# Entscheider/depthhead

Hardware: NVIDIA B200
Metric: frames/s, 640x480 depth, 10 trees depth 15, stride 5 (higher is better)
Workload: dtype f64

## Files before the change

depthhead_b200/api.py:

```python
from __future__ import annotations

import ctypes as C
from dataclasses import dataclass

import numpy as np

from . import capi


class IntrinsicMatrix:

    def __init__(self, mat):
        m = np.asarray(mat, np.float32)
        if m.size != 9:
            raise ValueError("IntrinsicMatrix needs 9 values")
        self.mat = np.ascontiguousarray(m.reshape(3, 3))

    @staticmethod
    def default_kinect_intrinsic() -> "IntrinsicMatrix":
        return IntrinsicMatrix([[560.0, 0.0, 320.0], [0.0, 560.0, 240.0], [0.0, 0.0, 1.0]])

    def _ptr(self):
        return capi.ptr(self.mat)

# ... 49 lines not shown
    def stage_ms(self) -> dict:
        a = np.zeros(capi.DH_N_STAGES, np.float32)
        capi.check(capi.load().dh_ctx_stage_ms(self._h, capi.ptr(a)))
        return dict(zip(capi.STAGES, a.tolist()))

    def counters(self) -> dict:
        a = np.zeros(capi.DH_N_COUNTERS, np.uint64)
        capi.check(capi.load().dh_ctx_counters(self._h, capi.ptr(a)))
        return dict(zip(capi.COUNTERS, (int(x) for x in a)))

    def tile_plan(self) -> dict:
        v = np.zeros(8, np.uint32)
        capi.check(capi.load().dh_debug_tile_plan(self._h, capi.ptr(v)))
        keys = ("patches_x", "patches_y", "tiles_x", "tiles_y", "tile_w", "tile_h", "smem_bytes", "threads")
        return {k: int(x) for k, x in zip(keys, v)}

    def debug_dims(self):
        a, b, c = C.c_uint32(), C.c_uint32(), C.c_uint32()
        capi.check(capi.load().dh_debug_dims(self._h, C.byref(a), C.byref(b), C.byref(c)))
        return a.value, b.value, c.value

    def debug_leaf_indices(self) -> np.ndarray:
        npx, npy, T = self.debug_dims()
        out = np.zeros((npx * npy, T), np.int32)
        capi.check(capi.load().dh_debug_leaf_indices(self._h, capi.ptr(out)))
        return out

    def debug_patches(self):
        npx, npy, _ = self.debug_dims()
        p3 = np.zeros((npx * npy, 3), np.float32)
# ... 250 lines not shown
```

depthhead_b200/capi.py:

```python
from __future__ import annotations

import ctypes as C
import os

import numpy as np

from . import _build

DH_OK, DH_E_JSON, DH_E_SHAPE, DH_E_CUDA, DH_E_ARG, DH_E_STATE = 0, -1, -2, -3, -4, -5
DH_DEPTH_HOST, DH_DEPTH_DEVICE = 0, 1
DH_N_STAGES, DH_N_COUNTERS = 7, 12
STAGES = ("h2d", "sat", "traverse", "gate", "vote", "meanshift", "d2h")
COUNTERS = ("frames", "patches", "valid_patches", "evals", "node_visits", "gate_patches", "hits",
            "centre_votes", "rot_votes", "launches", "meanshift_iters", "cube_rebuilds")


class DhError(RuntimeError):
    def __init__(self, code: int, msg: str):
        super().__init__("%s (code %d)" % (msg, code))
        self.code = code


class dh_result(C.Structure):
    _fields_ = [("mid_point", C.c_float * 3), ("_pad", C.c_uint32), ("rotation", C.c_double * 3),
# ... 78 lines not shown
    "dh_hough_image_raw": (C.c_int, [_vp, _vp, _vp, _u32, _u32, _vp, _vp]),
    "dh_build_hough_image": (C.c_int, [_vp, _vp, _vp, _u32, _u32, _vp, _vp]),
    "dh_predict_from2dhough": (C.c_int, [_vp, _vp, _vp, _u32, _u32, _vp, C.POINTER(dh_result)]),
    "dh_ctx_enable_stage_timing": (C.c_int, [_vp, C.c_int]),
    "dh_ctx_stage_ms": (C.c_int, [_vp, _vp]),
    "dh_ctx_counters": (C.c_int, [_vp, _vp]),
    "dh_ctx_enable_debug": (C.c_int, [_vp, C.c_int]),
    "dh_debug_dims": (C.c_int, [_vp, C.POINTER(_u32), C.POINTER(_u32), C.POINTER(_u32)]),
    "dh_debug_leaf_indices": (C.c_int, [_vp, _vp]),
    "dh_debug_patches": (C.c_int, [_vp, _vp, _vp]),
    "dh_debug_seeds": (C.c_int, [_vp, _vp, _vp, _vp, _vp]),
    "dh_debug_votes": (C.c_int, [_vp, C.c_int, _vp, _vp, C.POINTER(_u64), _vp, C.POINTER(_i32)]),
    "dh_debug_meanshift": (C.c_int, [_vp, C.c_int, _vp, C.POINTER(_u32)]),
    "dh_debug_meanshift_flags": (C.c_int, [_vp, _vp]),
    "dh_debug_tile_plan": (C.c_int, [_vp, _vp]),
    "dh_debug_leaf_static": (C.c_int, [_vp, _vp, _vp, _vp, _vp]),
}

_lib = None


def lib_path() -> str:
    return _build.LIB


def load():
    global _lib
    if _lib is not None:
        return _lib
    if os.environ.get("DH_NO_BUILD") != "1":
# ... 25 lines not shown
```

depthhead_b200/csrc/dh_capi.cu:

```cuda
#include <cstring>
#include <memory>
#include <new>
#include <algorithm>
#include <string>
#include <vector>

#include "../../include/depthhead_cuda.h"
#include "dh_ctx.hpp"
#include "dh_forest.hpp"
#include "dh_json.hpp"

struct dh_forest {
    std::unique_ptr<dh::HostForest> hf;
};
struct dh_ctx {
    std::unique_ptr<dh::Context> cx;
};

namespace {

thread_local std::string g_last_error = "";

int fail(int code, const std::string& msg) {
    g_last_error = msg;
// ... 273 lines not shown
int dh_train_split_level(dh_ctx* c, const dh_trainset* t, const uint32_t* sample_idx, const uint64_t* node_off, uint32_t n_nodes,
                         const int32_t* rects, const double* thr, uint8_t* bits) {
    return guarded([&] {
        REQUIRE(c && t && node_off && (n_nodes == 0 || (sample_idx && rects && thr && bits)), "dh_train_split_level: NULL argument");
        c->cx->train_split_level(*t->ts, sample_idx, node_off, n_nodes, rects, thr, bits);
    });
}
int dh_debug_tile_plan(dh_ctx* c, uint32_t plan[8]) {
    return guarded([&] {
        REQUIRE(c && plan, "dh_debug_tile_plan: NULL argument");
        const dh::TilePlan& t = c->cx->tile_plan();
        const uint32_t v[8] = {t.tpx, t.tpy, t.tiles_x, t.tiles_y, t.tw, t.th, t.smem_bytes, t.threads};
        std::memcpy(plan, v, sizeof(v));
    });
}
int dh_train_forest(dh_ctx* c, const dh_train_params* p, const uint16_t* patches, uint64_t n, const uint8_t* is_object,
                    const float* offsets, const double* rotations, dh_forest** out) {
    return guarded([&] {
        REQUIRE(c && p && patches && is_object && offsets && rotations && out, "dh_train_forest: NULL argument");
        *out = nullptr;
        std::unique_ptr<dh::HostForest> hf(c->cx->train_forest(*p, patches, n, is_object, offsets, rotations));
        *out = new dh_forest{std::move(hf)};
    });
}
int dh_train_learn(dh_ctx* c, const dh_train_params* p, uint32_t n_frames, uint32_t w, uint32_t h, const uint16_t* depth,
                   const uint8_t* mask, const float* K, const float* pos3d, const float* rot, dh_forest** out) {
    return guarded([&] {
        REQUIRE(c && p && out && (n_frames == 0 || (depth && mask && K && pos3d && rot)), "dh_train_learn: NULL argument");
        *out = nullptr;
        std::unique_ptr<dh::HostForest> hf(c->cx->train_learn(*p, n_frames, w, h, depth, mask, K, pos3d, rot));
// ... 131 lines not shown
```

depthhead_b200/csrc/dh_ctx.cu:

```cuda
#include "dh_ctx.hpp"

#include <algorithm>
#include <atomic>
#include <chrono>
#include <cmath>
#include <cstdio>
#include <cstdlib>
#include <cstring>
#include <thread>

namespace dh {

#define DH_CUDA(expr)                                                                                   \
    do {                                                                                                \
        cudaError_t _e = (expr);                                                                        \
        if (_e != cudaSuccess)                                                                          \
            throw ModelError(DH_E_CUDA, std::string(#expr) + ": " + cudaGetErrorString(_e));            \
    } while (0)

namespace {

template <typename T>
void dev_alloc(T*& p, size_t n) {
    p = nullptr;
// ... 61 lines not shown
    }
    DH_CUDA(cudaStreamCreateWithFlags(&copy_stream2_, cudaStreamNonBlocking));
    for (int i = 0; i < kStageSlots; ++i) {
        DH_CUDA(cudaEventCreateWithFlags(&ev_copied_[i], cudaEventDisableTiming));
        DH_CUDA(cudaEventCreateWithFlags(&ev_consumed_[i], cudaEventDisableTiming));
    }
    dev_alloc(d_counters_, DH_N_COUNTERS);
    DH_CUDA(cudaHostAlloc((void**)&h_fs_, sizeof(FrameState), cudaHostAllocDefault));
    DH_CUDA(cudaHostAlloc((void**)&h_counters_, sizeof(unsigned long long) * DH_N_COUNTERS, cudaHostAllocDefault));
    DH_CUDA(cudaHostAlloc((void**)&h_result1_, sizeof(dh_result), cudaHostAllocDefault));
    for (int i = 0; i < kEncSlots; ++i) DH_CUDA(cudaEventCreateWithFlags(&ev_enc_copied_[i], cudaEventDisableTiming));
    DH_CUDA(cudaEventCreateWithFlags(&ev_copy_tail_, cudaEventDisableTiming));
    if (const char* v = std::getenv("DH_HOST_ENCODE")) host_encode_ = *v ? (int)std::strtol(v, nullptr, 10) : -1;
    use_graphs_ = env_flag("DH_GRAPH", true);
    cube_clear_fused_ = env_flag("DH_CUBE_CLEAR_FUSED", true);
    gate_split_ = env_flag("DH_GATE_SPLIT", true);
    gate_split_min_ = env_u32("DH_GATE_SPLIT_MIN", 64);
    chunk_frames_ = env_u32("DH_CHUNK_FRAMES", 0);
    debug_sync_ = env_u32("DH_DEBUG_SYNC", 0) != 0;
    std::memset(stage_ms_, 0, sizeof(stage_ms_));
    std::memset(counters_, 0, sizeof(counters_));
}

Context::~Context() {
    cudaSetDevice(device_);
    cudaDeviceSynchronize();
    drop_graph();
    free_scratch();
    free_forest();
    dev_free(d_counters_);
// ... 272 lines not shown
    fdev_.pair_leaf_perm = df_pair_perm_;
    fdev_.leaf_prob = df_leaf_prob_;
    fdev_.leaf_info = df_leaf_info_;
    fdev_.offsets = df_offsets_;
    fdev_.rot_bins = df_rot_bins_;
    fdev_.rot_cells = df_rot_cells_;
    fdev_.leaf_box = df_leaf_box_;
    fdev_.ms_kernel = df_kernel_;
    fdev_.n_trees = hf.n_trees;
}

void Context::free_lane(Lane& L) {
    dev_free(L.sat);
    dev_free(L.band_u);
    dev_free(L.box);
    dev_free(L.leaf);
    dev_free(L.p3);
    dev_free(L.gate);
    dev_free(L.gated);
    dev_free(L.cubes);
    dev_free(L.grids);
    dev_free(L.fs);
    dev_free(L.results);
    dev_free(L.ms_trace);
    L.allocated = false;
    L.cubes_clean = false;
}

void Context::drop_graph() {
    if (graph_exec_) cudaGraphExecDestroy(graph_exec_);
// ... 21 lines not shown
        if (w + 1 <= 1024 && env_flag("DH_SAT_BANDS", true))
            dev_alloc(L.band_u, F * (size_t)((h + sat_band_rows() - 1) / sat_band_rows()) * (w + 1));
    }
    dev_alloc(L.leaf, F * P * T);
    dev_alloc(L.p3, F * P * 3);
    dev_alloc(L.gate, F * P);
    dev_alloc(L.gated, F * P);
    dev_alloc(L.cubes, F * 2 * (size_t)vote_box_cells());
    DH_CUDA(cudaMemsetAsync(L.cubes, 0, sizeof(uint32_t) * F * 2 * (size_t)vote_box_cells(), stream_));
    L.cubes_clean = true;
    dev_alloc(L.grids, F * (size_t)(kPosGridCells + kRotGridCells));
    dev_alloc(L.fs, F);
    dev_alloc(L.results, F);
    if (sk_.trace_iters) dev_alloc(L.ms_trace, F * 2 * (size_t)sk_.trace_iters * 3);
    if (g.P) {
        const cuuint64_t gdim[3] = {(cuuint64_t)(g.rw ? g.box_w : w + 1), (cuuint64_t)(g.rw ? g.box_h : h + 1), (cuuint64_t)F};
        const cuuint64_t row_bytes = (cuuint64_t)(g.rw ? g.box_pitch : g.sat_pitch) * 4u;
        const cuuint64_t gstr[2] = {row_bytes, row_bytes * (g.rw ? g.box_h : h + 1)};
        const cuuint32_t box[3] = {tiles_.tw, tiles_.th, 1u};
        const cuuint32_t estr[3] = {1u, 1u, 1u};
        CUresult r = get_encode_fn()(&L.sat_map, CU_TENSOR_MAP_DATA_TYPE_UINT32, 3, g.rw ? L.box : L.sat, gdim, gstr, box, estr,
                                     CU_TENSOR_MAP_INTERLEAVE_NONE, CU_TENSOR_MAP_SWIZZLE_NONE,
                                     CU_TENSOR_MAP_L2_PROMOTION_L2_128B, CU_TENSOR_MAP_FLOAT_OOB_FILL_NONE);
        if (r != CUDA_SUCCESS) throw ModelError(DH_E_CUDA, "cuTensorMapEncodeTiled failed with code " + std::to_string((int)r));
    }
    DH_CUDA(cudaStreamSynchronize(stream_));
    L.allocated = true;
}

TilePlan Context::plan_tiles(const Geometry& g) const {
// ... 124 lines not shown
        DH_CUDA(cudaStreamSynchronize(copy_stream_));
        DH_CUDA(cudaStreamSynchronize(copy_stream2_));
        for (int i = 0; i < kStageSlots; ++i) dev_free(d_depth_[i]);
        staging_elems_ = n;
    }
    for (int i = 0; i < slots && i < kStageSlots; ++i)
        if (!d_depth_[i]) dev_alloc(d_depth_[i], staging_elems_);
}

FrameBuffers Context::buffers(const Lane& L, const uint16_t* depth) const {
    FrameBuffers b{};
    b.depth = depth;
    b.sat = L.sat;
    b.band_u = L.band_u;
    b.box = L.box;
    b.leaf = L.leaf;
    b.p3 = debug_ ? L.p3 : nullptr;
    b.gate = debug_ ? L.gate : nullptr;
    b.gated = L.gated;
    b.grids = L.grids;
    b.fs = L.fs;
    b.cubes = L.cubes;
    b.results = L.results;
    b.ms_trace = L.ms_trace;
    b.ms_trace_cap = sk_.trace_iters;
    b.leaf_mask = leaf_codes_ ? kLeafIdMask : 0x7fffffffu;
    b.debug = debug_ ? 1u : 0u;
    b.clear_cubes = (!debug_ && cube_clear_fused_) ? 1u : 0u;
    return b;
}
// ... 36 lines not shown
    if (g.P && hot_tw_ != tiles_.tw) {
        launch_plan_nodes(df_nodes_, df_hot_, df_uni_, df_n_nodes_, tiles_.tw, leaf_codes_ ? df_leaf_prob_ : nullptr, stream_);
        if (df_pair_recs_) launch_plan_pairs(df_pair_topo_, df_uni_, df_pair_recs_, df_n_pairs_, stream_);
        DH_CUDA(cudaStreamSynchronize(stream_));
        hot_tw_ = tiles_.tw;
    }
    mark(DH_STAGE_SAT);
    launches_ += (uint64_t)(g.rw ? launch_box_image(b, g, n, n_sms_, st) : launch_sat(b, g, n, st));
    stage_check("sat");
    mark(DH_STAGE_TRAVERSE);
    if (g.P) {
        if (debug_)
            DH_CUDA(cudaMemsetAsync(L.leaf, 0xFF, sizeof(int32_t) * (size_t)n * g.n_trees * g.P, st));
        else
            DH_CUDA(cudaMemset2DAsync(L.leaf, sizeof(int32_t) * (size_t)g.n_trees * g.P, 0xFF, sizeof(int32_t) * (size_t)g.P, n, st));
        launch_traverse(L.sat_map, b, g, tiles_, fdev_, n, st);
        launches_ += 1;
        stage_check("traverse");
    }
}

void Context::run_back(Lane& L, const FrameBuffers& b, uint32_t n, uint32_t iterations) {
    const Geometry& g = geom_;
    cudaStream_t st = L.stream;
    mark(DH_STAGE_GATE);
    launches_ += (uint64_t)launch_gate_coarse(b, g, fdev_, n, gate_split_ && n >= gate_split_min_, n_sms_, st);
    stage_check("gate + coarse grids");
    mark(DH_STAGE_VOTE);
    if (iterations && !L.cubes_clean) DH_CUDA(cudaMemsetAsync(L.cubes, 0, sizeof(uint32_t) * 2 * (size_t)vote_box_cells() * n, st));
    if (iterations) L.cubes_clean = false;
    launches_ += (uint64_t)launch_seed_and_cubes(b, g, fdev_, n, iterations, st);
    stage_check("seeds + accumulator cubes");
// ... 706 lines not shown
    if (npx) *npx = geom_.npx;
    if (npy) *npy = geom_.npy;
    if (n_trees) *n_trees = geom_.n_trees;
}
void Context::debug_leaf(int32_t* leaf) {
    require_debug();
    const size_t P = geom_.P, T = geom_.n_trees;
    std::vector<int32_t> tmp(P * T);
    DH_CUDA(cudaMemcpy(tmp.data(), lanes_[0].leaf, P * T * sizeof(int32_t), cudaMemcpyDeviceToHost));
    for (size_t t = 0; t < T; ++t)
        for (size_t p = 0; p < P; ++p) {
            const int32_t w = tmp[t * P + p];
            leaf[p * T + t] = (w >= 0 && leaf_codes_) ? (int32_t)((uint32_t)w & kLeafIdMask) : w;
        }
}
void Context::debug_patches(float* p3, uint8_t* gate) {
    require_debug();
    const size_t P = geom_.P;
    if (gate) DH_CUDA(cudaMemcpy(gate, lanes_[0].gate, P, cudaMemcpyDeviceToHost));
    if (p3) DH_CUDA(cudaMemcpy(p3, lanes_[0].p3, P * 3 * sizeof(float), cudaMemcpyDeviceToHost));
}
void Context::debug_seeds(uint32_t* guess_pos, uint32_t* guess_rot, int32_t* seed_mid, int32_t* seed_rot) {
    require_debug();
    if (guess_pos) DH_CUDA(cudaMemcpy(guess_pos, lanes_[0].grids, kPosGridCells * sizeof(uint32_t), cudaMemcpyDeviceToHost));
    if (guess_rot) DH_CUDA(cudaMemcpy(guess_rot, lanes_[0].grids + kPosGridCells, kRotGridCells * sizeof(uint32_t), cudaMemcpyDeviceToHost));
    FrameState fs;
    DH_CUDA(cudaMemcpy(&fs, lanes_[0].fs, sizeof(fs), cudaMemcpyDeviceToHost));
    for (int k = 0; k < 3; ++k) {
        if (seed_mid) seed_mid[k] = fs.seed_mid[k];
        if (seed_rot) seed_rot[k] = fs.seed_rot[k];
// ... 61 lines not shown
```

depthhead_b200/csrc/dh_ctx.hpp:

```cpp
#pragma once

#include <cuda.h>
#include <cuda_runtime.h>

#include <cstdint>
#include <cstring>
#include <memory>
#include <utility>
#include <vector>

#include "dh_forest.hpp"
#include "dh_hostenc.hpp"
#include "dh_kernels.cuh"

namespace dh {

struct Lane {
    cudaStream_t stream = nullptr;
    cudaStream_t own = nullptr;
    cudaEvent_t done = nullptr;
    uint32_t* sat = nullptr;
    uint32_t* band_u = nullptr;
    uint32_t* box = nullptr;
    int32_t* leaf = nullptr;
    float* p3 = nullptr;
    uint8_t* gate = nullptr;
    float4* gated = nullptr;
    uint32_t* grids = nullptr;
    FrameState* fs = nullptr;
    dh_result* results = nullptr;
    int32_t* ms_trace = nullptr;
    uint32_t* cubes = nullptr;
    CUtensorMap sat_map{};
    bool allocated = false;
    bool cubes_clean = false;
};
constexpr int kMaxLanes = 4;

// ... 49 lines not shown
    void train_split_level(const TrainSet& ts, const uint32_t* sample_idx, const uint64_t* node_off, uint32_t n_nodes,
                           const int32_t* rects, const double* thr, uint8_t* bits);
    void predict_mask(const HostForest& hf, const uint16_t* depth, uint32_t w, uint32_t h, uint8_t* mask);
    void hough_image_raw(const HostForest& hf, const uint16_t* depth, uint32_t w, uint32_t h, const float K[9],
                         uint16_t* votes);
    void hough_image(const HostForest& hf, const uint16_t* depth, uint32_t w, uint32_t h, const float K[9], uint16_t* votes,
                     bool blur, dh_result* from2d);

    void debug_dims(uint32_t* npx, uint32_t* npy, uint32_t* n_trees) const;
    void debug_leaf(int32_t* leaf);
    void debug_patches(float* p3, uint8_t* gate);
    void debug_seeds(uint32_t* guess_pos, uint32_t* guess_rot, int32_t* seed_mid, int32_t* seed_rot);
    void debug_votes(int which, int32_t* keys, uint32_t* vals, uint64_t* n, int32_t* box_origin, int32_t* box_dim);
    void debug_meanshift(int which, int32_t* pos, uint32_t* n_iter);
    void debug_leaf_static(const HostForest& hf, uint32_t* valtoadd, uint8_t* rot_ok, uint8_t* off_ok);
    uint32_t last_ms_flags(int which) const { return last_ms_flags_[which & 1]; }
    const TilePlan& tile_plan() const { return tiles_; }

private:
    void ensure_forest(const HostForest& hf);
    void free_forest();
    void build_pair_tables(const HostForest& hf, const std::vector<int32_t>& dev_index);
    void ensure_scratch(const HostForest& hf, uint32_t w, uint32_t h, uint32_t n_frames_hint, const float K[9], int n_lanes = 1);
    void alloc_lane(Lane& L);
    void free_lane(Lane& L);
    void ensure_staging(int slots);
    void ensure_biwi(const uint64_t* offsets, uint32_t n, uint32_t chunk, int slots);
    void check_biwi_status(uint32_t n);
    void run_batch(const HostForest& hf, const uint16_t* depth, const uint8_t* blob, const uint64_t* offsets, uint32_t n, uint32_t w,
                   uint32_t h, const float K[9], int depth_loc, dh_result* out);
// ... 103 lines not shown
                   iterations == o.iterations && std::memcmp(K, o.K, sizeof(K)) == 0 && stream == o.stream && depth == o.depth &&
                   scratch == o.scratch && result == o.result;
        }
    };
    void drop_graph();
    cudaGraphExec_t graph_exec_ = nullptr;
    GraphKey graph_key_{}, graph_seen_{};
    bool graph_seen_valid_ = false;
    uint64_t graph_launches_ = 0;
    bool use_graphs_ = true;
    bool prob_codes_ok_ = false;
    bool leaf_codes_ = false;
    uint32_t gate_split_min_ = 64;
    bool gate_split_ = true;
    bool cube_clear_fused_ = true;

    bool timing_ = false, debug_ = false, have_debug_ = false, debug_sync_ = false;
    uint32_t debug_iterations_ = 0;
    uint32_t last_ms_flags_[2] = {0, 0};
    std::vector<cudaEvent_t> timing_events_;
    size_t ev_used_ = 0;
    std::vector<std::pair<int, cudaEvent_t>> marks_;
    std::vector<std::pair<cudaEvent_t, cudaEvent_t>> copy_marks_;
    float stage_ms_[DH_N_STAGES];
    uint64_t counters_[DH_N_COUNTERS];
    uint64_t launches_ = 0;
};

}
```

depthhead_b200/csrc/dh_kernels.cu:

```cuda
#include "dh_kernels.cuh"

#include <algorithm>
#include <atomic>
#include <cstdio>
#include <cstdlib>

namespace dh {

namespace dev {

__device__ __forceinline__ uint32_t smem_u32(const void* p) { return (uint32_t)__cvta_generic_to_shared(p); }

__device__ __forceinline__ void fence_mbar_init() {
    asm volatile("fence.mbarrier_init.release.cluster;" ::: "memory");
}
__device__ __forceinline__ void prefetch_tensormap(const CUtensorMap* map) {
    asm volatile("prefetch.tensormap [%0];" ::"l"(map) : "memory");
}

__device__ __forceinline__ void img_to_space(const float* Kinv, float x, float y, float z, float out[3]) {
    float r[3];
#pragma unroll
    for (int j = 0; j < 3; ++j) {
        float t = __fmul_rn(x, Kinv[j * 3 + 0]);
// ... 442 lines not shown
    asm volatile("st.shared.u32 [%0], %1;" ::"r"(addr), "r"(v) : "memory");
}
__device__ __forceinline__ void sts_u16(uint32_t addr, uint32_t v) {
    asm volatile("st.shared.u16 [%0], %1;" ::"r"(addr), "h"((uint16_t)v) : "memory");
}

__device__ __noinline__ bool binarize_ieee(const NodeRec* __restrict__ nodes, int32_t node, uint32_t s1, uint32_t s2) {
    const NodeRec r = nodes[node];
    const uint32_t c1 = (uint32_t)(r.r[2] - r.r[0]) * (uint32_t)(r.r[3] - r.r[1]);
    const uint32_t c2 = (uint32_t)(r.r[6] - r.r[4]) * (uint32_t)(r.r[7] - r.r[5]);
    const double avg1 = c1 ? __ddiv_rn(__uint2double_rn(s1), __uint2double_rn(c1)) : 0.0;
    const double avg2 = c2 ? __ddiv_rn(__uint2double_rn(s2), __uint2double_rn(c2)) : 0.0;
    return __dsub_rn(avg1, avg2) > r.threshold;
}

template <int kThreads, int kMode>
__global__ void __launch_bounds__(kThreads, kThreads >= 768 ? 2 : 3) traverse_kernel(const __grid_constant__ CUtensorMap sat_map,
                                                            cudaTextureObject_t hot_tex,
                                                            const HotNode* __restrict__ hot,
                                                            const UniNode* __restrict__ uni,
                                                            const NodeRec* __restrict__ nodes,
                                                            const int32_t* __restrict__ roots, int32_t* __restrict__ leaf,
                                                            const uint32_t* __restrict__ sat,
                                                            FrameState* __restrict__ fs, Geometry g, TilePlan tp,
                                                            uint32_t uni_rw, uint32_t uni_rh, const PairRec* __restrict__ pair_recs,
                                                            const int32_t* __restrict__ pair_roots, const int32_t* __restrict__ pair_perm) {
    extern __shared__ uint8_t smem_raw[];
    const uint32_t tile_a = (smem_u32(smem_raw) + 127u) & ~127u;
    const uint32_t tile_bytes = tp.tw * tp.th * 4u;
    const uint32_t bar_a = tile_a + ((tile_bytes + 15u) & ~15u);
    const uint32_t live_a = bar_a + 16u;
    __shared__ uint32_t s_nlive, s_empty;

    const uint32_t frame = blockIdx.y;
    const uint32_t tile_x = blockIdx.x % tp.tiles_x, tile_y = blockIdx.x / tp.tiles_x;
    const uint32_t px0 = tile_x * tp.tpx, py0 = tile_y * tp.tpy;
    const uint32_t tid = threadIdx.x;
    const uint32_t npt = tp.tpx * tp.tpy;
    const int T = (int)g.n_trees;
    int32_t* leaf_f = leaf + (size_t)frame * T * g.P;

    const uint32_t x0 = px0 * g.stride, y0 = py0 * g.stride, ax0 = x0 & ~3u, dx = x0 - ax0;
    if (tid == 0) {
        prefetch_tensormap(&sat_map);
        asm volatile("mbarrier.init.shared::cta.b64 [%0], %1;" ::"r"(bar_a), "r"(1u) : "memory");
        fence_mbar_init();
        s_nlive = 0;
        if (tp.tma_first) {
            asm volatile("mbarrier.arrive.expect_tx.shared::cta.b64 _, [%0], %1;" ::"r"(bar_a), "r"(tile_bytes) : "memory");
            asm volatile(
                "cp.async.bulk.tensor.3d.shared::cluster.global.mbarrier::complete_tx::bytes [%0], [%1, {%2, %3, %4}], [%5];" ::"r"(tile_a),
                "l"(&sat_map), "r"((int)ax0), "r"((int)y0), "r"((int)frame), "r"(bar_a)
                : "memory");
        }
    }
    if (tid < 32u) {
        const uint32_t lastx = min(px0 + tp.tpx, g.npx) - 1u, lasty = min(py0 + tp.tpy, g.npy) - 1u;
        const uint32_t x1 = lastx * g.stride + g.sw, y1 = lasty * g.stride + g.sh;
        bool any;
        if (kMode >= 4) {
            const uint32_t nkx = (x1 - x0 + uni_rw - 1u) / uni_rw, nky = (y1 - y0 + uni_rh - 1u) / uni_rh;
            const uint32_t* B = sat + (size_t)frame * g.box_h * g.box_pitch;
            uint32_t acc = 0;
            for (uint32_t i = tid; i < nkx * nky; i += 32u) {
                const uint32_t kx = i % nkx, ky = i / nkx;
                const uint32_t bx = min(x0 + kx * uni_rw, x1 - uni_rw), by = min(y0 + ky * uni_rh, y1 - uni_rh);
                acc |= __ldg(B + (size_t)by * g.box_pitch + bx);
            }
            any = __any_sync(0xffffffffu, acc != 0u);
        } else {
            const uint32_t* S = sat + (size_t)frame * (g.h + 1) * g.sat_pitch;
            const uint32_t sum = __ldg(S + (size_t)y1 * g.sat_pitch + x1) - __ldg(S + (size_t)y0 * g.sat_pitch + x1) -
                                 __ldg(S + (size_t)y1 * g.sat_pitch + x0) + __ldg(S + (size_t)y0 * g.sat_pitch + x0);
            any = sum != 0u;
        }
        if (tid == 0) {
            s_empty = !any;
            if (any && !tp.tma_first) {
                asm volatile("mbarrier.arrive.expect_tx.shared::cta.b64 _, [%0], %1;" ::"r"(bar_a), "r"(tile_bytes) : "memory");
                asm volatile(
                    "cp.async.bulk.tensor.3d.shared::cluster.global.mbarrier::complete_tx::bytes [%0], [%1, {%2, %3, %4}], [%5];" ::"r"(tile_a),
                    "l"(&sat_map), "r"((int)ax0), "r"((int)y0), "r"((int)frame), "r"(bar_a)
                    : "memory");
            }
        }
    }
    __syncthreads();
    if (s_empty && !tp.tma_first) return;
    {
        asm volatile(
            "{\n"
            ".reg .pred P1;\n"
            "LAB_WAIT:\n"
            "mbarrier.try_wait.parity.shared::cta.b64 P1, [%0], %1;\n"
            "@P1 bra DONE;\n"
            "bra LAB_WAIT;\n"
            "DONE:\n"
            "}\n" ::"r"(bar_a),
            "r"(0u)
            : "memory");
    }
    if (s_empty) return;

    const uint32_t tw4 = tp.tw * 4u;
    const uint32_t org_a = tile_a + dx * 4u;
    const uint32_t nbx = (tp.tpx + 7u) >> 3;
    const uint32_t n_lp = tp.blocked ? nbx * ((tp.tpy + 3u) >> 2) * 32u : ((npt + 31u) & ~31u);
    for (uint32_t lp = tid; lp < n_lp; lp += kThreads) {
        bool ok = false;
        uint32_t packed = 0;
        uint32_t lx, ly;
        if (tp.blocked) {
            const uint32_t blk = lp >> 5;
            lx = (blk % nbx) * 8u + (lp & 7u);
            ly = (blk / nbx) * 4u + ((lp >> 3) & 3u);
        } else {
            lx = lp % tp.tpx;
// ... 1622 lines not shown
    static SmemConfig configured;
    if (configured.raise(tp.smem_bytes)) {
        cudaFuncSetAttribute(traverse_kernel<kThreads, 0>, cudaFuncAttributeMaxDynamicSharedMemorySize, (int)tp.smem_bytes);
        cudaFuncSetAttribute(traverse_kernel<kThreads, 1>, cudaFuncAttributeMaxDynamicSharedMemorySize, (int)tp.smem_bytes);
        cudaFuncSetAttribute(traverse_kernel<kThreads, 2>, cudaFuncAttributeMaxDynamicSharedMemorySize, (int)tp.smem_bytes);
        cudaFuncSetAttribute(traverse_kernel<kThreads, 3>, cudaFuncAttributeMaxDynamicSharedMemorySize, (int)tp.smem_bytes);
        cudaFuncSetAttribute(traverse_kernel<kThreads, 4>, cudaFuncAttributeMaxDynamicSharedMemorySize, (int)tp.smem_bytes);
        cudaFuncSetAttribute(traverse_kernel<kThreads, 5>, cudaFuncAttributeMaxDynamicSharedMemorySize, (int)tp.smem_bytes);
        cudaFuncSetAttribute(traverse_kernel<kThreads, 6>, cudaFuncAttributeMaxDynamicSharedMemorySize, (int)tp.smem_bytes);
        cudaFuncSetAttribute(traverse_kernel<kThreads, 7>, cudaFuncAttributeMaxDynamicSharedMemorySize, (int)tp.smem_bytes);
    }
    static const bool two_walks = std::getenv("DH_TRAV_ILP") && std::atoi(std::getenv("DH_TRAV_ILP")) == 2;
    dim3 gr(tp.tiles_x * tp.tiles_y, n_frames);
    if (f.uni && g.rw && f.pair_recs)
        traverse_kernel<kThreads, 7><<<gr, kThreads, tp.smem_bytes, s>>>(sat_map, f.hot_tex, f.hot, f.uni, f.nodes, f.roots, b.leaf, b.box,
                                                                       b.fs, g, tp, f.uni_rw, f.uni_rh, f.pair_recs, f.pair_roots, f.pair_leaf_perm);
    else if (f.uni && g.rw && f.hot_tex && two_walks)
        traverse_kernel<kThreads, 6><<<gr, kThreads, tp.smem_bytes, s>>>(sat_map, f.hot_tex, f.hot, f.uni, f.nodes, f.roots, b.leaf, b.box,
                                                                       b.fs, g, tp, f.uni_rw, f.uni_rh, f.pair_recs, f.pair_roots, f.pair_leaf_perm);
    else if (f.uni && g.rw && f.hot_tex)
        traverse_kernel<kThreads, 4><<<gr, kThreads, tp.smem_bytes, s>>>(sat_map, f.hot_tex, f.hot, f.uni, f.nodes, f.roots, b.leaf, b.box,
                                                                       b.fs, g, tp, f.uni_rw, f.uni_rh, f.pair_recs, f.pair_roots, f.pair_leaf_perm);
    else if (f.uni && g.rw)
        traverse_kernel<kThreads, 5><<<gr, kThreads, tp.smem_bytes, s>>>(sat_map, 0, f.hot, f.uni, f.nodes, f.roots, b.leaf, b.box, b.fs, g,
                                                                       tp, f.uni_rw, f.uni_rh, f.pair_recs, f.pair_roots, f.pair_leaf_perm);
    else if (f.uni && f.hot_tex)
        traverse_kernel<kThreads, 2><<<gr, kThreads, tp.smem_bytes, s>>>(sat_map, f.hot_tex, f.hot, f.uni, f.nodes, f.roots, b.leaf, b.sat,
                                                                       b.fs, g, tp, f.uni_rw, f.uni_rh, f.pair_recs, f.pair_roots, f.pair_leaf_perm);
    else if (f.uni)
        traverse_kernel<kThreads, 3><<<gr, kThreads, tp.smem_bytes, s>>>(sat_map, 0, f.hot, f.uni, f.nodes, f.roots, b.leaf, b.sat, b.fs, g,
                                                                       tp, f.uni_rw, f.uni_rh, f.pair_recs, f.pair_roots, f.pair_leaf_perm);
    else if (f.hot_tex)
        traverse_kernel<kThreads, 1><<<gr, kThreads, tp.smem_bytes, s>>>(sat_map, f.hot_tex, f.hot, f.uni, f.nodes, f.roots, b.leaf, b.sat,
                                                                       b.fs, g, tp, 0u, 0u, nullptr, nullptr, nullptr);
    else
        traverse_kernel<kThreads, 0><<<gr, kThreads, tp.smem_bytes, s>>>(sat_map, 0, f.hot, f.uni, f.nodes, f.roots, b.leaf, b.sat, b.fs, g,
                                                                       tp, 0u, 0u, nullptr, nullptr, nullptr);
}

void launch_traverse(const CUtensorMap& sat_map, const FrameBuffers& b, const Geometry& g, const TilePlan& tp,
                     const ForestDev& f, uint32_t n_frames, cudaStream_t s) {
    if (tp.threads >= 1024) launch_traverse_t<1024>(sat_map, b, g, tp, f, n_frames, s);
    else if (tp.threads >= 768) launch_traverse_t<768>(sat_map, b, g, tp, f, n_frames, s);
    else launch_traverse_t<512>(sat_map, b, g, tp, f, n_frames, s);
}

void launch_plan_nodes(const NodeRec* nodes, HotNode* hot, UniNode* uni, size_t n_nodes, uint32_t tile_width,
                       const double* prob_codes, cudaStream_t s) {
    if (n_nodes == 0) return;
    plan_nodes_kernel<<<(unsigned)((n_nodes + 255) / 256), 256, 0, s>>>(nodes, hot, uni, n_nodes, tile_width, prob_codes);
}

void launch_plan_pairs(const PairTopo* topo, const UniNode* uni, PairRec* recs, size_t n_recs, cudaStream_t s) {
    if (n_recs == 0) return;
    plan_pairs_kernel<<<(unsigned)((n_recs + 255) / 256), 256, 0, s>>>(topo, uni, recs, n_recs);
}

uint32_t sat_band_rows() { return (uint32_t)kSatBandRows; }
uint32_t vote_box_cells() { return (uint32_t)kBoxCells; }
// ... 110 lines not shown
```

depthhead_b200/csrc/dh_kernels.cuh:

```cuda
#pragma once

#include <cuda.h>
#include <cuda_runtime.h>

#include <cstdint>

#include "dh_types.hpp"
#include "../../include/depthhead_cuda.h"

namespace dh {

struct alignas(16) FrameState {
    uint32_t n_chits;
    uint32_t n_rhits;
    uint32_t n_valid;
    uint32_t n_gate;
    unsigned long long n_mid_votes;
    unsigned long long n_rot_votes;
    unsigned long long node_visits;
    int32_t seed_mid[3];
    int32_t seed_rot[3];
    uint32_t ms_iters[2];
    uint32_t ms_flags[2];
    uint32_t rebuilds[2];
    int32_t box_org[2][3];
    uint32_t box_valid[2];
    uint32_t has_guess;
    float midp_guess[3];
    double rot_guess[3];
    uint32_t work_next;
    uint32_t _pad[3];
};

struct Geometry {
    uint32_t w, h;
    uint32_t sw, sh;
    uint32_t left_w, left_h;
    uint32_t stride;
    uint32_t npx, npy, P;
    uint32_t sat_pitch;
    uint32_t n_trees;
    uint32_t magic_w, magic_h;
    uint32_t rw, rh;
    uint32_t box_w, box_h;
    uint32_t box_pitch;
    float K[9], Kinv[9];
// ... 27 lines not shown
    const double* leaf_prob;
    const LeafInfo* leaf_info;
    const float4* offsets;
    const uint32_t* rot_bins;
    const uint32_t* rot_cells;
    const LeafBox* leaf_box;
    const float* ms_kernel;
    int32_t n_trees;
};

struct FrameBuffers {
    const uint16_t* depth;
    uint32_t* sat;
    uint32_t* band_u;
    uint32_t* box;
    int32_t* leaf;
    float* p3;
    uint8_t* gate;
    float4* gated;
    uint32_t* grids;
    FrameState* fs;
    uint32_t* cubes;
    dh_result* results;
    int32_t* ms_trace;
    uint32_t ms_trace_cap;
    uint32_t leaf_mask;
    uint32_t debug;
    uint32_t clear_cubes;
};

constexpr uint32_t kProbCodeShift = 23u;
constexpr uint32_t kLeafIdMask = (1u << kProbCodeShift) - 1u;

int launch_sat(const FrameBuffers& b, const Geometry& g, uint32_t n_frames, cudaStream_t s);
int launch_box_image(const FrameBuffers& b, const Geometry& g, uint32_t n_frames, int n_sms, cudaStream_t s);
bool box_image_supported(uint32_t w, uint32_t h, uint32_t sw, uint32_t sh, uint32_t rw, uint32_t rh);
void launch_traverse(const CUtensorMap& sat_map, const FrameBuffers& b, const Geometry& g, const TilePlan& tp,
                     const ForestDev& f, uint32_t n_frames, cudaStream_t s);
void launch_plan_nodes(const NodeRec* nodes, HotNode* hot, UniNode* uni, size_t n_nodes, uint32_t tile_width,
                       const double* prob_codes, cudaStream_t s);
void launch_plan_pairs(const PairTopo* topo, const UniNode* uni, PairRec* recs, size_t n_recs, cudaStream_t s);
int launch_gate_coarse(const FrameBuffers& b, const Geometry& g, const ForestDev& f, uint32_t n_frames, bool from_list, int n_sms,
                       cudaStream_t s);
int launch_seed_and_cubes(const FrameBuffers& b, const Geometry& g, const ForestDev& f, uint32_t n_frames,
                          uint32_t iterations, cudaStream_t s);
int launch_meanshift(const FrameBuffers& b, const Geometry& g, const ForestDev& f, uint32_t n_frames, uint32_t iterations,
                     int n_sms, cudaStream_t s);
uint32_t sat_band_rows();
uint32_t vote_box_cells();
uint32_t vote_box_dim();
void launch_leaf_gates(const double* leaf_prob, const uint32_t* vote_start, const uint32_t* n_votes,
                       const float* offsets, const double* rotations, const uint32_t* rot_bins, LeafInfo* out,
                       LeafBox* box_out, uint32_t* rot_cells, uint32_t n_leaves, cudaStream_t s);
// ... 19 lines not shown
```

include/depthhead_cuda.h:

```cpp
#ifndef DEPTHHEAD_CUDA_H
#define DEPTHHEAD_CUDA_H

#include <stddef.h>
#include <stdint.h>

#ifdef __cplusplus
extern "C" {
#endif

#define DH_ABI_VERSION 1

#define DH_OK 0
#define DH_E_JSON (-1)
#define DH_E_SHAPE (-2)
#define DH_E_CUDA (-3)
#define DH_E_ARG (-4)
#define DH_E_STATE (-5)

typedef struct dh_forest dh_forest;
typedef struct dh_ctx dh_ctx;

typedef struct dh_result {
    float mid_point[3];
    uint32_t _pad;
// ... 120 lines not shown
int dh_ctx_enable_stage_timing(dh_ctx* c, int on);
int dh_ctx_stage_ms(dh_ctx* c, float ms[DH_N_STAGES]);
#define DH_N_COUNTERS 12
int dh_ctx_counters(dh_ctx* c, uint64_t counters[DH_N_COUNTERS]);

int dh_ctx_enable_debug(dh_ctx* c, int on);
int dh_debug_dims(dh_ctx* c, uint32_t* npx, uint32_t* npy, uint32_t* n_trees);
int dh_debug_leaf_indices(dh_ctx* c, int32_t* leaf );
int dh_debug_patches(dh_ctx* c, float* p3, uint8_t* gate);
int dh_debug_seeds(dh_ctx* c, uint32_t* guess_pos, uint32_t* guess_rot, int32_t seed_mid[3], int32_t seed_rot[3]);
int dh_debug_votes(dh_ctx* c, int which, int32_t* keys , uint32_t* vals, uint64_t* n,
                   int32_t box_origin[3], int32_t* box_dim);
int dh_debug_meanshift(dh_ctx* c, int which, int32_t* pos , uint32_t* n_iter);
int dh_debug_meanshift_flags(dh_ctx* c, uint32_t flags[2]);
int dh_debug_tile_plan(dh_ctx* c, uint32_t plan[8]);
int dh_debug_leaf_static(dh_ctx* c, const dh_forest* f, uint32_t* valtoadd, uint8_t* rot_ok, uint8_t* off_ok);

#ifdef __cplusplus
}
#endif
#endif
```

Baseline: 435,900.

## Compact non-empty tiles in a pre-pass before traverse

Adds a small warp-per-tile kernel that tests each tile window for any valid depth and appends live tile ids to a per-frame list, using an atomic counter in FrameState. The traverse kernel then maps its blocks onto this compacted list. Blocks past the live count exit immediately, and live blocks start their TMA tile load without doing the in-kernel emptiness check first. The cost is one extra launch per chunk, a list buffer, and a per-frame counter that must be reset correctly between frames. A debug API for reading the live-tile list is also added.

```diff
diff --git a/depthhead_b200/api.py b/depthhead_b200/api.py
--- a/depthhead_b200/api.py
+++ b/depthhead_b200/api.py
@@ -87,6 +87,13 @@
         capi.check(capi.load().dh_debug_tile_plan(self._h, capi.ptr(v)))
         keys = ("patches_x", "patches_y", "tiles_x", "tiles_y", "tile_w", "tile_h", "smem_bytes", "threads")
         return {k: int(x) for k, x in zip(keys, v)}
+
+    def debug_live_tiles(self) -> np.ndarray:
+        tp = self.tile_plan()
+        out = np.zeros(max(1, tp["tiles_x"] * tp["tiles_y"]), np.uint32)
+        n = C.c_uint32()
+        capi.check(capi.load().dh_debug_live_tiles(self._h, C.byref(n), capi.ptr(out)))
+        return np.sort(out[:n.value])
 
     def debug_dims(self):
         a, b, c = C.c_uint32(), C.c_uint32(), C.c_uint32()
diff --git a/depthhead_b200/capi.py b/depthhead_b200/capi.py
--- a/depthhead_b200/capi.py
+++ b/depthhead_b200/capi.py
@@ -116,6 +116,7 @@
     "dh_debug_meanshift": (C.c_int, [_vp, C.c_int, _vp, C.POINTER(_u32)]),
     "dh_debug_meanshift_flags": (C.c_int, [_vp, _vp]),
     "dh_debug_tile_plan": (C.c_int, [_vp, _vp]),
+    "dh_debug_live_tiles": (C.c_int, [_vp, C.POINTER(_u32), _vp]),
     "dh_debug_leaf_static": (C.c_int, [_vp, _vp, _vp, _vp, _vp]),
 }
 
diff --git a/depthhead_b200/csrc/dh_capi.cu b/depthhead_b200/csrc/dh_capi.cu
--- a/depthhead_b200/csrc/dh_capi.cu
+++ b/depthhead_b200/csrc/dh_capi.cu
@@ -311,6 +311,12 @@
         std::memcpy(plan, v, sizeof(v));
     });
 }
+int dh_debug_live_tiles(dh_ctx* c, uint32_t* n, uint32_t* tiles) {
+    return guarded([&] {
+        REQUIRE(c && n, "dh_debug_live_tiles: NULL argument");
+        c->cx->debug_live_tiles(n, tiles);
+    });
+}
 int dh_train_forest(dh_ctx* c, const dh_train_params* p, const uint16_t* patches, uint64_t n, const uint8_t* is_object,
                     const float* offsets, const double* rotations, dh_forest** out) {
     return guarded([&] {
diff --git a/depthhead_b200/csrc/dh_ctx.cu b/depthhead_b200/csrc/dh_ctx.cu
--- a/depthhead_b200/csrc/dh_ctx.cu
+++ b/depthhead_b200/csrc/dh_ctx.cu
@@ -99,6 +99,7 @@
     if (const char* v = std::getenv("DH_HOST_ENCODE")) host_encode_ = *v ? (int)std::strtol(v, nullptr, 10) : -1;
     use_graphs_ = env_flag("DH_GRAPH", true);
     cube_clear_fused_ = env_flag("DH_CUBE_CLEAR_FUSED", true);
+    live_tiles_ = env_flag("DH_LIVE_TILES", true);
     gate_split_ = env_flag("DH_GATE_SPLIT", true);
     gate_split_min_ = env_u32("DH_GATE_SPLIT_MIN", 64);
     chunk_frames_ = env_u32("DH_CHUNK_FRAMES", 0);
@@ -401,6 +402,7 @@
     dev_free(L.sat);
     dev_free(L.band_u);
     dev_free(L.box);
+    dev_free(L.live);
     dev_free(L.leaf);
     dev_free(L.p3);
     dev_free(L.gate);
@@ -452,6 +454,7 @@
     dev_alloc(L.results, F);
     if (sk_.trace_iters) dev_alloc(L.ms_trace, F * 2 * (size_t)sk_.trace_iters * 3);
     if (g.P) {
+        dev_alloc(L.live, F * tiles_.tiles_x * tiles_.tiles_y);
         const cuuint64_t gdim[3] = {(cuuint64_t)(g.rw ? g.box_w : w + 1), (cuuint64_t)(g.rw ? g.box_h : h + 1), (cuuint64_t)F};
         const cuuint64_t row_bytes = (cuuint64_t)(g.rw ? g.box_pitch : g.sat_pitch) * 4u;
         const cuuint64_t gstr[2] = {row_bytes, row_bytes * (g.rw ? g.box_h : h + 1)};
@@ -606,6 +609,7 @@
     b.sat = L.sat;
     b.band_u = L.band_u;
     b.box = L.box;
+    b.live = live_tiles_ ? L.live : nullptr;
     b.leaf = L.leaf;
     b.p3 = debug_ ? L.p3 : nullptr;
     b.gate = debug_ ? L.gate : nullptr;
@@ -672,8 +676,7 @@
             DH_CUDA(cudaMemsetAsync(L.leaf, 0xFF, sizeof(int32_t) * (size_t)n * g.n_trees * g.P, st));
         else
             DH_CUDA(cudaMemset2DAsync(L.leaf, sizeof(int32_t) * (size_t)g.n_trees * g.P, 0xFF, sizeof(int32_t) * (size_t)g.P, n, st));
-        launch_traverse(L.sat_map, b, g, tiles_, fdev_, n, st);
-        launches_ += 1;
+        launches_ += (uint64_t)launch_traverse(L.sat_map, b, g, tiles_, fdev_, n, st);
         stage_check("traverse");
     }
 }
@@ -1410,6 +1413,14 @@
             leaf[p * T + t] = (w >= 0 && leaf_codes_) ? (int32_t)((uint32_t)w & kLeafIdMask) : w;
         }
 }
+void Context::debug_live_tiles(uint32_t* n, uint32_t* tiles) {
+    require_debug();
+    if (!live_tiles_) throw ModelError(DH_E_STATE, "no live-tile lists: DH_LIVE_TILES=0");
+    uint32_t count = 0;
+    if (geom_.P) DH_CUDA(cudaMemcpy(&count, &lanes_[0].fs->n_live_tiles, sizeof(count), cudaMemcpyDeviceToHost));
+    if (n) *n = count;
+    if (tiles && count) DH_CUDA(cudaMemcpy(tiles, lanes_[0].live, count * sizeof(uint32_t), cudaMemcpyDeviceToHost));
+}
 void Context::debug_patches(float* p3, uint8_t* gate) {
     require_debug();
     const size_t P = geom_.P;
diff --git a/depthhead_b200/csrc/dh_ctx.hpp b/depthhead_b200/csrc/dh_ctx.hpp
--- a/depthhead_b200/csrc/dh_ctx.hpp
+++ b/depthhead_b200/csrc/dh_ctx.hpp
@@ -22,6 +22,7 @@
     uint32_t* sat = nullptr;
     uint32_t* band_u = nullptr;
     uint32_t* box = nullptr;
+    uint32_t* live = nullptr;
     int32_t* leaf = nullptr;
     float* p3 = nullptr;
     uint8_t* gate = nullptr;
@@ -101,6 +102,7 @@
     void debug_votes(int which, int32_t* keys, uint32_t* vals, uint64_t* n, int32_t* box_origin, int32_t* box_dim);
     void debug_meanshift(int which, int32_t* pos, uint32_t* n_iter);
     void debug_leaf_static(const HostForest& hf, uint32_t* valtoadd, uint8_t* rot_ok, uint8_t* off_ok);
+    void debug_live_tiles(uint32_t* n, uint32_t* tiles);
     uint32_t last_ms_flags(int which) const { return last_ms_flags_[which & 1]; }
     const TilePlan& tile_plan() const { return tiles_; }
 
@@ -234,6 +236,7 @@
     uint32_t gate_split_min_ = 64;
     bool gate_split_ = true;
     bool cube_clear_fused_ = true;
+    bool live_tiles_ = true;
 
     bool timing_ = false, debug_ = false, have_debug_ = false, debug_sync_ = false;
     uint32_t debug_iterations_ = 0;
diff --git a/depthhead_b200/csrc/dh_kernels.cu b/depthhead_b200/csrc/dh_kernels.cu
--- a/depthhead_b200/csrc/dh_kernels.cu
+++ b/depthhead_b200/csrc/dh_kernels.cu
@@ -480,6 +480,55 @@
     return __dsub_rn(avg1, avg2) > r.threshold;
 }
 
+template <bool kBox>
+__device__ __forceinline__ bool tile_window_any(const uint32_t* __restrict__ src, const Geometry& g, const TilePlan& tp, uint32_t rw,
+                                                uint32_t rh, uint32_t frame, uint32_t px0, uint32_t py0, uint32_t lane) {
+    const uint32_t x0 = px0 * g.stride, y0 = py0 * g.stride;
+    const uint32_t lastx = min(px0 + tp.tpx, g.npx) - 1u, lasty = min(py0 + tp.tpy, g.npy) - 1u;
+    const uint32_t x1 = lastx * g.stride + g.sw, y1 = lasty * g.stride + g.sh;
+    if (kBox) {
+        const uint32_t nkx = (x1 - x0 + rw - 1u) / rw, nky = (y1 - y0 + rh - 1u) / rh;
+        const uint32_t* B = src + (size_t)frame * g.box_h * g.box_pitch;
+        auto tap = [&](uint32_t i) {
+            const uint32_t kx = i % nkx, ky = i / nkx;
+            const uint32_t bx = min(x0 + kx * rw, x1 - rw), by = min(y0 + ky * rh, y1 - rh);
+            return __ldg(B + (size_t)by * g.box_pitch + bx);
+        };
+        uint32_t acc = 0;
+        for (uint32_t i = lane; i < nkx * nky; i += 64u) {
+            const uint32_t a = tap(i), b = i + 32u < nkx * nky ? tap(i + 32u) : 0u;
+            acc |= a | b;
+        }
+        return __any_sync(0xffffffffu, acc != 0u);
+    }
+    const uint32_t* S = src + (size_t)frame * (g.h + 1) * g.sat_pitch;
+    const uint32_t sum = __ldg(S + (size_t)y1 * g.sat_pitch + x1) - __ldg(S + (size_t)y0 * g.sat_pitch + x1) -
+                         __ldg(S + (size_t)y1 * g.sat_pitch + x0) + __ldg(S + (size_t)y0 * g.sat_pitch + x0);
+    return sum != 0u;
+}
+
+constexpr int kLiveWarps = 8;
+template <bool kBox>
+__global__ void __launch_bounds__(kLiveWarps * 32) live_tiles_kernel(const uint32_t* __restrict__ src, FrameState* __restrict__ fs,
+                                                                     uint32_t* __restrict__ live, Geometry g, TilePlan tp,
+                                                                     uint32_t n_frames) {
+    const uint32_t n_tiles = tp.tiles_x * tp.tiles_y;
+    const uint32_t wid = blockIdx.x * kLiveWarps + (threadIdx.x >> 5), lane = threadIdx.x & 31u;
+    const uint32_t frame = wid / n_tiles, tile = wid - frame * n_tiles;
+    if (frame >= n_frames) return;
+    const uint32_t px0 = (tile % tp.tiles_x) * tp.tpx, py0 = (tile / tp.tiles_x) * tp.tpy;
+    if (tile_window_any<kBox>(src, g, tp, g.rw, g.rh, frame, px0, py0, lane) && lane == 0u)
+        live[(size_t)frame * n_tiles + atomicAdd(&fs[frame].n_live_tiles, 1u)] = tile;
+}
+
+__device__ __forceinline__ void tma_tile_load(uint32_t dst, const CUtensorMap* map, uint32_t x, uint32_t y, uint32_t frame, uint32_t bar,
+                                              uint32_t bytes) {
+    asm volatile("mbarrier.arrive.expect_tx.shared::cta.b64 _, [%0], %1;" ::"r"(bar), "r"(bytes) : "memory");
+    asm volatile("cp.async.bulk.tensor.3d.shared::cluster.global.mbarrier::complete_tx::bytes [%0], [%1, {%2, %3, %4}], [%5];" ::"r"(dst),
+                 "l"(map), "r"((int)x), "r"((int)y), "r"((int)frame), "r"(bar)
+                 : "memory");
+}
+
 template <int kThreads, int kMode>
 __global__ void __launch_bounds__(kThreads, kThreads >= 768 ? 2 : 3) traverse_kernel(const __grid_constant__ CUtensorMap sat_map,
                                                             cudaTextureObject_t hot_tex,
@@ -490,7 +539,8 @@
                                                             const uint32_t* __restrict__ sat,
                                                             FrameState* __restrict__ fs, Geometry g, TilePlan tp,
                                                             uint32_t uni_rw, uint32_t uni_rh, const PairRec* __restrict__ pair_recs,
-                                                            const int32_t* __restrict__ pair_roots, const int32_t* __restrict__ pair_perm) {
+                                                            const int32_t* __restrict__ pair_roots, const int32_t* __restrict__ pair_perm,
+                                                            const uint32_t* __restrict__ live) {
     extern __shared__ uint8_t smem_raw[];
     const uint32_t tile_a = (smem_u32(smem_raw) + 127u) & ~127u;
     const uint32_t tile_bytes = tp.tw * tp.th * 4u;
@@ -498,8 +548,15 @@
     const uint32_t live_a = bar_a + 16u;
     __shared__ uint32_t s_nlive, s_empty;
 
+    const uint32_t n_tiles = tp.tiles_x * tp.tiles_y;
     const uint32_t frame = blockIdx.y;
-    const uint32_t tile_x = blockIdx.x % tp.tiles_x, tile_y = blockIdx.x / tp.tiles_x;
+    uint32_t tile = blockIdx.x;
+    if (live) {
+        const uint32_t n_live = fs[frame].n_live_tiles, listed = live[(size_t)frame * n_tiles + tile];
+        if ((tile >= n_live) | (listed >= n_tiles)) return;
+        tile = listed;
+    }
+    const uint32_t tile_x = tile % tp.tiles_x, tile_y = tile / tp.tiles_x;
     const uint32_t px0 = tile_x * tp.tpx, py0 = tile_y * tp.tpy;
     const uint32_t tid = threadIdx.x;
     const uint32_t npt = tp.tpx * tp.tpy;
@@ -512,47 +569,17 @@
         asm volatile("mbarrier.init.shared::cta.b64 [%0], %1;" ::"r"(bar_a), "r"(1u) : "memory");
         fence_mbar_init();
         s_nlive = 0;
-        if (tp.tma_first) {
-            asm volatile("mbarrier.arrive.expect_tx.shared::cta.b64 _, [%0], %1;" ::"r"(bar_a), "r"(tile_bytes) : "memory");
-            asm volatile(
-                "cp.async.bulk.tensor.3d.shared::cluster.global.mbarrier::complete_tx::bytes [%0], [%1, {%2, %3, %4}], [%5];" ::"r"(tile_a),
-                "l"(&sat_map), "r"((int)ax0), "r"((int)y0), "r"((int)frame), "r"(bar_a)
-                : "memory");
-        }
-    }
-    if (tid < 32u) {
-        const uint32_t lastx = min(px0 + tp.tpx, g.npx) - 1u, lasty = min(py0 + tp.tpy, g.npy) - 1u;
-        const uint32_t x1 = lastx * g.stride + g.sw, y1 = lasty * g.stride + g.sh;
-        bool any;
-        if (kMode >= 4) {
-            const uint32_t nkx = (x1 - x0 + uni_rw - 1u) / uni_rw, nky = (y1 - y0 + uni_rh - 1u) / uni_rh;
-            const uint32_t* B = sat + (size_t)frame * g.box_h * g.box_pitch;
-            uint32_t acc = 0;
-            for (uint32_t i = tid; i < nkx * nky; i += 32u) {
-                const uint32_t kx = i % nkx, ky = i / nkx;
-                const uint32_t bx = min(x0 + kx * uni_rw, x1 - uni_rw), by = min(y0 + ky * uni_rh, y1 - uni_rh);
-                acc |= __ldg(B + (size_t)by * g.box_pitch + bx);
-            }
-            any = __any_sync(0xffffffffu, acc != 0u);
-        } else {
-            const uint32_t* S = sat + (size_t)frame * (g.h + 1) * g.sat_pitch;
-            const uint32_t sum = __ldg(S + (size_t)y1 * g.sat_pitch + x1) - __ldg(S + (size_t)y0 * g.sat_pitch + x1) -
-                                 __ldg(S + (size_t)y1 * g.sat_pitch + x0) + __ldg(S + (size_t)y0 * g.sat_pitch + x0);
-            any = sum != 0u;
-        }
+        if (live || tp.tma_first) tma_tile_load(tile_a, &sat_map, ax0, y0, frame, bar_a, tile_bytes);
+    }
+    if (!live && tid < 32u) {
+        const bool any = tile_window_any<(kMode >= 4)>(sat, g, tp, uni_rw, uni_rh, frame, px0, py0, tid);
         if (tid == 0) {
             s_empty = !any;
-            if (any && !tp.tma_first) {
-                asm volatile("mbarrier.arrive.expect_tx.shared::cta.b64 _, [%0], %1;" ::"r"(bar_a), "r"(tile_bytes) : "memory");
-                asm volatile(
-                    "cp.async.bulk.tensor.3d.shared::cluster.global.mbarrier::complete_tx::bytes [%0], [%1, {%2, %3, %4}], [%5];" ::"r"(tile_a),
-                    "l"(&sat_map), "r"((int)ax0), "r"((int)y0), "r"((int)frame), "r"(bar_a)
-                    : "memory");
-            }
+            if (any && !tp.tma_first) tma_tile_load(tile_a, &sat_map, ax0, y0, frame, bar_a, tile_bytes);
         }
     }
     __syncthreads();
-    if (s_empty && !tp.tma_first) return;
+    if (!live && s_empty && !tp.tma_first) return;
     {
         asm volatile(
             "{\n"
@@ -566,7 +593,7 @@
             "r"(0u)
             : "memory");
     }
-    if (s_empty) return;
+    if (!live && s_empty) return;
 
     const uint32_t tw4 = tp.tw * 4u;
     const uint32_t org_a = tile_a + dx * 4u;
@@ -2219,35 +2246,43 @@
     dim3 gr(tp.tiles_x * tp.tiles_y, n_frames);
     if (f.uni && g.rw && f.pair_recs)
         traverse_kernel<kThreads, 7><<<gr, kThreads, tp.smem_bytes, s>>>(sat_map, f.hot_tex, f.hot, f.uni, f.nodes, f.roots, b.leaf, b.box,
-                                                                       b.fs, g, tp, f.uni_rw, f.uni_rh, f.pair_recs, f.pair_roots, f.pair_leaf_perm);
+                                                                       b.fs, g, tp, f.uni_rw, f.uni_rh, f.pair_recs, f.pair_roots, f.pair_leaf_perm, b.live);
     else if (f.uni && g.rw && f.hot_tex && two_walks)
         traverse_kernel<kThreads, 6><<<gr, kThreads, tp.smem_bytes, s>>>(sat_map, f.hot_tex, f.hot, f.uni, f.nodes, f.roots, b.leaf, b.box,
-                                                                       b.fs, g, tp, f.uni_rw, f.uni_rh, f.pair_recs, f.pair_roots, f.pair_leaf_perm);
+                                                                       b.fs, g, tp, f.uni_rw, f.uni_rh, f.pair_recs, f.pair_roots, f.pair_leaf_perm, b.live);
     else if (f.uni && g.rw && f.hot_tex)
         traverse_kernel<kThreads, 4><<<gr, kThreads, tp.smem_bytes, s>>>(sat_map, f.hot_tex, f.hot, f.uni, f.nodes, f.roots, b.leaf, b.box,
-                                                                       b.fs, g, tp, f.uni_rw, f.uni_rh, f.pair_recs, f.pair_roots, f.pair_leaf_perm);
+                                                                       b.fs, g, tp, f.uni_rw, f.uni_rh, f.pair_recs, f.pair_roots, f.pair_leaf_perm, b.live);
     else if (f.uni && g.rw)
         traverse_kernel<kThreads, 5><<<gr, kThreads, tp.smem_bytes, s>>>(sat_map, 0, f.hot, f.uni, f.nodes, f.roots, b.leaf, b.box, b.fs, g,
-                                                                       tp, f.uni_rw, f.uni_rh, f.pair_recs, f.pair_roots, f.pair_leaf_perm);
+                                                                       tp, f.uni_rw, f.uni_rh, f.pair_recs, f.pair_roots, f.pair_leaf_perm, b.live);
     else if (f.uni && f.hot_tex)
         traverse_kernel<kThreads, 2><<<gr, kThreads, tp.smem_bytes, s>>>(sat_map, f.hot_tex, f.hot, f.uni, f.nodes, f.roots, b.leaf, b.sat,
-                                                                       b.fs, g, tp, f.uni_rw, f.uni_rh, f.pair_recs, f.pair_roots, f.pair_leaf_perm);
+                                                                       b.fs, g, tp, f.uni_rw, f.uni_rh, f.pair_recs, f.pair_roots, f.pair_leaf_perm, b.live);
     else if (f.uni)
         traverse_kernel<kThreads, 3><<<gr, kThreads, tp.smem_bytes, s>>>(sat_map, 0, f.hot, f.uni, f.nodes, f.roots, b.leaf, b.sat, b.fs, g,
-                                                                       tp, f.uni_rw, f.uni_rh, f.pair_recs, f.pair_roots, f.pair_leaf_perm);
+                                                                       tp, f.uni_rw, f.uni_rh, f.pair_recs, f.pair_roots, f.pair_leaf_perm, b.live);
     else if (f.hot_tex)
         traverse_kernel<kThreads, 1><<<gr, kThreads, tp.smem_bytes, s>>>(sat_map, f.hot_tex, f.hot, f.uni, f.nodes, f.roots, b.leaf, b.sat,
-                                                                       b.fs, g, tp, 0u, 0u, nullptr, nullptr, nullptr);
+                                                                       b.fs, g, tp, 0u, 0u, nullptr, nullptr, nullptr, b.live);
     else
         traverse_kernel<kThreads, 0><<<gr, kThreads, tp.smem_bytes, s>>>(sat_map, 0, f.hot, f.uni, f.nodes, f.roots, b.leaf, b.sat, b.fs, g,
-                                                                       tp, 0u, 0u, nullptr, nullptr, nullptr);
-}
-
-void launch_traverse(const CUtensorMap& sat_map, const FrameBuffers& b, const Geometry& g, const TilePlan& tp,
-                     const ForestDev& f, uint32_t n_frames, cudaStream_t s) {
+                                                                       tp, 0u, 0u, nullptr, nullptr, nullptr, b.live);
+}
+
+int launch_traverse(const CUtensorMap& sat_map, const FrameBuffers& b, const Geometry& g, const TilePlan& tp,
+                    const ForestDev& f, uint32_t n_frames, cudaStream_t s) {
+    int launches = 1;
+    if (b.live) {
+        const uint32_t blocks = (uint32_t)(((uint64_t)tp.tiles_x * tp.tiles_y * n_frames + kLiveWarps - 1) / kLiveWarps);
+        if (g.rw) live_tiles_kernel<true><<<blocks, kLiveWarps * 32, 0, s>>>(b.box, b.fs, b.live, g, tp, n_frames);
+        else live_tiles_kernel<false><<<blocks, kLiveWarps * 32, 0, s>>>(b.sat, b.fs, b.live, g, tp, n_frames);
+        ++launches;
+    }
     if (tp.threads >= 1024) launch_traverse_t<1024>(sat_map, b, g, tp, f, n_frames, s);
     else if (tp.threads >= 768) launch_traverse_t<768>(sat_map, b, g, tp, f, n_frames, s);
     else launch_traverse_t<512>(sat_map, b, g, tp, f, n_frames, s);
+    return launches;
 }
 
 void launch_plan_nodes(const NodeRec* nodes, HotNode* hot, UniNode* uni, size_t n_nodes, uint32_t tile_width,
diff --git a/depthhead_b200/csrc/dh_kernels.cuh b/depthhead_b200/csrc/dh_kernels.cuh
--- a/depthhead_b200/csrc/dh_kernels.cuh
+++ b/depthhead_b200/csrc/dh_kernels.cuh
@@ -29,7 +29,8 @@
     float midp_guess[3];
     double rot_guess[3];
     uint32_t work_next;
-    uint32_t _pad[3];
+    uint32_t n_live_tiles;
+    uint32_t _pad[2];
 };
 
 struct Geometry {
@@ -87,6 +88,7 @@
     uint32_t* sat;
     uint32_t* band_u;
     uint32_t* box;
+    uint32_t* live;
     int32_t* leaf;
     float* p3;
     uint8_t* gate;
@@ -108,8 +110,8 @@
 int launch_sat(const FrameBuffers& b, const Geometry& g, uint32_t n_frames, cudaStream_t s);
 int launch_box_image(const FrameBuffers& b, const Geometry& g, uint32_t n_frames, int n_sms, cudaStream_t s);
 bool box_image_supported(uint32_t w, uint32_t h, uint32_t sw, uint32_t sh, uint32_t rw, uint32_t rh);
-void launch_traverse(const CUtensorMap& sat_map, const FrameBuffers& b, const Geometry& g, const TilePlan& tp,
-                     const ForestDev& f, uint32_t n_frames, cudaStream_t s);
+int launch_traverse(const CUtensorMap& sat_map, const FrameBuffers& b, const Geometry& g, const TilePlan& tp,
+                    const ForestDev& f, uint32_t n_frames, cudaStream_t s);
 void launch_plan_nodes(const NodeRec* nodes, HotNode* hot, UniNode* uni, size_t n_nodes, uint32_t tile_width,
                        const double* prob_codes, cudaStream_t s);
 void launch_plan_pairs(const PairTopo* topo, const UniNode* uni, PairRec* recs, size_t n_recs, cudaStream_t s);
diff --git a/include/depthhead_cuda.h b/include/depthhead_cuda.h
--- a/include/depthhead_cuda.h
+++ b/include/depthhead_cuda.h
@@ -158,6 +158,7 @@
 int dh_debug_meanshift(dh_ctx* c, int which, int32_t* pos , uint32_t* n_iter);
 int dh_debug_meanshift_flags(dh_ctx* c, uint32_t flags[2]);
 int dh_debug_tile_plan(dh_ctx* c, uint32_t plan[8]);
+int dh_debug_live_tiles(dh_ctx* c, uint32_t* n, uint32_t* tiles );
 int dh_debug_leaf_static(dh_ctx* c, const dh_forest* f, uint32_t* valtoadd, uint8_t* rot_ok, uint8_t* off_ok);
 
 #ifdef __cplusplus
```

Measured after the change: 446,900 (median of 6 runs). 2.5% higher.
